# sadPororo/AD-YOLO

Hardware: AMD Instinct MI355X
Metric: train-step audio-sec/s (4ch, se-resnet34+adyolo) (higher is better)
Workload: dtype f32; 1 GPU; se-resnet34 + adyolo loss, synthetic 4ch 24kHz 60s clips, bs=64 per GPU, 12 classes, features+fwd+loss+bwd+allreduce+Adam; global_batch=64, parallelism=dp1

## Files before the change

ad-yolo_amd/_lib.py:

```python
import ctypes
import os

_HERE = os.path.dirname(os.path.abspath(__file__))
LIB_PATH = os.environ.get("ADYOLO_LIB") or os.path.join(_HERE, "libadyolo_hip.so")

P = ctypes.c_void_p
I = ctypes.c_int
L = ctypes.c_long
F = ctypes.c_float
U64 = ctypes.c_uint64

SIGNATURES = {
    "adyolo_abi_version": (I, []),
    "adyolo_last_error": (ctypes.c_char_p, []),
    "adyolo_feat_stft_mel": (I, [P] * 8 + [I, I] + [P] * 4 + [I, I, I, P]),
    "adyolo_feat_finish": (I, [P] * 4 + [I, I, I, P]),
    "adyolo_feat_gcc_phat": (I, [P] * 6 + [I, I, I, I, P]),
    "adyolo_nchw_to_nhwc8": (I, [P, P, I, I, I, I, P]),
    "adyolo_pack_w3x3": (I, [P, P, P, I, I, I, P]),
    "adyolo_conv3x3_tiles": (I, [I] * 3),
    "adyolo_conv3x3_fwd": (I, [P] * 13 + [I] * 7 + [P]),
    "adyolo_wino_pack_w": (I, [P, P, P, I, I, I, P]),
    "adyolo_wino_pack_many": (I, [P, I, I, I, P]),
    "adyolo_wino_tiles": (I, [I] * 3),
    "adyolo_wino_fwd": (I, [P] * 13 + [I] * 7 + [P]),
    "adyolo_wino4_pack_w": (I, [P, P, P, I, I, I, P]),
    "adyolo_wino4_pack_many": (I, [P, I, I, I, P]),
    "adyolo_wino4_tiles": (I, [I] * 3),
    "adyolo_wino4_fwd": (I, [P] * 13 + [I] * 7 + [P]),
    "adyolo_wino4_fwd_form": (I, [I] * 3),
    "adyolo_wino4_last_form": (I, []),
    "adyolo_set_switches": (I, [I]),
    "adyolo_wino4_wgrad_slabs": (I, [I] * 5),
    "adyolo_wino4_wgrad": (I, [P] * 7 + [I] * 6 + [P]),
    "adyolo_wino_wgrad_slabs": (I, [I] * 5),
    "adyolo_wino_wgrad": (I, [P] * 7 + [I] * 6 + [P]),
    "adyolo_conv3x3_wgrad_slabs": (I, [I] * 5),
    "adyolo_conv3x3_wgrad": (I, [P] * 6 + [I] * 6 + [P]),
    "adyolo_wgrad_plan": (I, [I] * 6 + [P]),
    "adyolo_conv_fwd_plan": (I, [I] * 9 + [P]),
    "adyolo_gemm": (I, [P] * 5 + [I] * 10 + [P]),
    "adyolo_gemm_plan": (I, [I] * 8 + [P, P, P]),
    "adyolo_gemm_batched": (I, [P] * 3 + [I] * 10 + [L] * 6 + [F, I, P]),
    "adyolo_colsum": (I, [P, P, P, I, I, I, I, P]),
    "adyolo_bn_stats": (I, [P] * 7 + [I, I, I, F, F, P]),
    "adyolo_bn_stats_tiles": (I, [P] * 11 + [I, I, I, I, F, F, P]),
    "adyolo_bn_eval_stats": (I, [P] * 4 + [I, F, P]),
    "adyolo_bn_scale_shift": (I, [P] * 6 + [I, P]),
    "adyolo_affine_nhwc": (I, [P] * 4 + [L, I, P]),
    "adyolo_bn_bwd_reduce": (I, [P] * 7 + [L, I, P]),
    "adyolo_bn_bwd_tiles": (I, [P, P, P, P, I, I, P]),
    "adyolo_bn_bwd_apply": (I, [P] * 12 + [L, I, I, F, P]),
    "adyolo_bn_persample": (I, [P, P, P, I, I, I, P]),
    "adyolo_bn_finish": (I, [P] * 10 + [I, I, I, F, F, P]),
    "adyolo_se_fc_fwd": (I, [P] * 10 + [I, I, I, I, P]),
    "adyolo_relu_mask_words": (L, [I, I, I]),
    "adyolo_se_tail_fwd": (I, [P] * 9 + [I, I, I, P]),
    "adyolo_se_tail_fwd_pool_ok": (I, [I, I, I]),
    "adyolo_se_tail_fwd_pool": (I, [P] * 9 + [I, I, I, I, P]),
    "adyolo_se_tail_bwd_reduce": (I, [P] * 9 + [I, I, I, P]),
    "adyolo_se_tail_bwd_tiles": (I, [P, P, P, I, I, I, P]),
    "adyolo_se_fc_bwd_words": (L, [I, I]),
    "adyolo_se_fc_bwd": (I, [P] * 16 + [I, I, I, I, P]),
    "adyolo_se_tail_bwd_apply": (I, [P] * 13 + [I, I, I, F, P]),
    "adyolo_se_tail_bwd_reduce_pooled": (I, [P] * 8 + [I, I, I, I, P]),
    "adyolo_se_tail_bwd_apply_pooled": (I, [P] * 13 + [I, I, I, I, F, P]),
    "adyolo_avgpool2_fwd": (I, [P, P, I, I, I, I, P]),
    "adyolo_avgpool2_bwd": (I, [P, P, I, I, I, I, P]),
    "adyolo_add": (I, [P, P, P, L, P]),
    "adyolo_mul": (I, [P, P, P, L, P]),
    "adyolo_scale_dev": (I, [P, P, P, L, P]),
    "adyolo_sap_fwd": (I, [P] * 5 + [I, I, I, P]),
    "adyolo_sap_bwd": (I, [P] * 8 + [I, I, I, P]),
    "adyolo_gru_fwd": (I, [P] * 6 + [I, I, P]),
    "adyolo_gru_bwd": (I, [P] * 6 + [I, I, P]),
    "adyolo_ln_tanh_fwd": (I, [P] * 4 + [L, I, F, P]),
    "adyolo_ln_tanh_bwd": (I, [P] * 8 + [L, I, F, P]),
    "adyolo_dropout_mask": (I, [P, L, F, U64, U64, P]),
    "adyolo_dropout_apply": (I, [P, P, L, F, U64, U64, P]),
    "adyolo_dropout_apply_dev": (I, [P, P, L, F, U64, U64, P, P]),
    "adyolo_counter_add": (I, [P, U64, P]),
    "adyolo_loss_workspace_words": (L, [I, I, I, I]),
    "adyolo_loss_fwd_bwd": (I, [P] * 6 + [I] * 7 + [P, P, F, F, F, F, P]),
    "adyolo_loss_phase": (I, [P] * 6 + [I] * 7 + [P, P, F, F, F, F, I, L, P]),
    "adyolo_loss_per_clip_workspace_words": (L, [I, I, I, I]),
    "adyolo_loss_per_clip": (I, [P] * 7 + [I] * 6 + [L, P, P, F, F, F, P]),
    "adyolo_loss_accumulate": (I, [P, P, I, P, P]),
    "adyolo_yolo_decode": (I, [P, P, L, I, I, I, I, F, F, F, P]),
    "adyolo_yolo_select_workspace_words": (L, [L, I, I]),
    "adyolo_yolo_select": (I, [P] * 4 + [L, I, I, F, F, F, F, I, P]),
    "adyolo_seld_score_workspace_words": (L, [L, I, I, I]),
# ... 120 lines not shown
```

ad-yolo_amd/csrc/conv.hip:

```cpp
#include <stdlib.h>
#include "common.hpp"

namespace adyolo {

template <int KC, int BN, int TW>
struct ConvCfg {
    static constexpr int TH = 256 / TW;
    static constexpr int HW_ = TW + 2;
    static constexpr int HH_ = TH + 2;
    static constexpr int NPIX = HW_ * HH_;
    static constexpr int AS = KC + 4;
    static constexpr int NT = BN / 32;
    static constexpr int Q = KC / 4;
    static constexpr int A_FLOATS = NPIX * AS;
    static constexpr int W_FLOATS = BN * AS;
    static constexpr int WPT = (BN * Q + 255) / 256;
};

template <int KC, int BN, int TW>
__global__ __launch_bounds__(256, 2) void conv3x3_fwd_kernel(
    const float *__restrict__ x, const float *__restrict__ wpk, const float *__restrict__ bias,
    const float *__restrict__ addend, const float *__restrict__ addend_mask, const float *__restrict__ in_scale,
    const float *__restrict__ in_shift, float *__restrict__ y, float *__restrict__ stats,
    const float *__restrict__ stat_aux, const float *__restrict__ stat_mean, const float *__restrict__ stat_invstd,
// ... 352 lines not shown
        f32x16 acc;
#pragma unroll
        for (int r = 0; r < 16; ++r) acc[r] = 0.f;
#pragma unroll
        for (int tap = 0; tap < 9; ++tap) {
            acc = mfma32(a[tap].x, bw[tap].x, acc);
            acc = mfma32(a[tap].y, bw[tap].y, acc);
            acc = mfma32(a[tap].z, bw[tap].z, acc);
            acc = mfma32(a[tap].w, bw[tap].w, acc);
        }
        if (gy < H) {
            float *ot = otile[wave];
#pragma unroll
            for (int r = 0; r < 16; ++r) {
                const int px = mfma_row(r, lane);
                float v = acc[r] + bv;
                if (relu) v = fmaxf(v, 0.f);
                ot[px * 36 + li] = v;
                if (tx0 + px < W) {
                    ssum += v;
                    float sq = v * v;
                    asm volatile("" : "+v"(sq));
                    ssq += sq;
                }
            }
            float *yrow = y + (((size_t)n * H + gy) * W + tx0) * 32;
#pragma unroll
            for (int k = 0; k < 4; ++k) {
                const int px = k * 8 + (lane >> 3), c4 = lane & 7;
                const f32x4 v4 = *reinterpret_cast<const f32x4 *>(&ot[px * 36 + c4 * 4]);
                if (tx0 + px < W) __builtin_nontemporal_store(v4, reinterpret_cast<f32x4 *>(yrow + (size_t)px * 32 + c4 * 4));
            }
        }
    }
    if (stats) {
        const float a0 = ssum + __shfl_xor(ssum, 32, 64), a1 = ssq + __shfl_xor(ssq, 32, 64);
        if (lh == 0) {
            red[(wave * 32 + li) * 2 + 0] = a0;
            red[(wave * 32 + li) * 2 + 1] = a1;
        }
        __syncthreads();
        if (tid < 64) {
            const int c = tid >> 1, which = tid & 1;
            const float v = red[(0 * 32 + c) * 2 + which] + red[(1 * 32 + c) * 2 + which] + red[(2 * 32 + c) * 2 + which] +
                            red[(3 * 32 + c) * 2 + which];
            stats[which * ((size_t)gridDim.x * 32) + (size_t)blockIdx.x * 32 + c] = v;
        }
    }
}

constexpr int SW_U = 8;
constexpr int SW_T = 64;
constexpr int SW_XS = (SW_T + 4) * 8;
__global__ __launch_bounds__(256, 2) void stem_wgrad_kernel(const float *__restrict__ x, const float *__restrict__ dy,
                                                            float *__restrict__ slabs, int H, int W, int rows_total) {
    __shared__ __attribute__((aligned(16))) float lds[4 * SW_T * 32 + 7 * SW_XS];
    static_assert(4 * SW_T * 32 + 7 * SW_XS >= 4 * 32 * 72, "the reduction buffer must fit");
    float *dyL = lds, *xL = lds + 4 * SW_T * 32;
    const int tid = threadIdx.x, lane = tid & 63, wave = tid >> 6;
    const int li = lane & 31, lh = lane >> 5;
    int ky[3], boff[3];
#pragma unroll
    for (int t = 0; t < 3; ++t) {
        const int n = t * 32 + li, tap = n < 72 ? n >> 3 : 8;
        ky[t] = tap / 3 - 1;
        boff[t] = (lh + 1 + (tap % 3 - 1)) * 8 + (n & 7);
    }
    f32x16 acc[3];
#pragma unroll
    for (int t = 0; t < 3; ++t)
#pragma unroll
        for (int r = 0; r < 16; ++r) acc[t][r] = 0.f;
    for (int i = tid; i < SW_XS; i += 256) xL[6 * SW_XS + i] = 0.f;

    const int per = (rows_total + gridDim.x - 1) / gridDim.x;
    const int r0 = blockIdx.x * per, r1 = min(rows_total, r0 + per);
    const int ncol = (W + SW_T - 1) / SW_T;
    const int nchunk = r0 < r1 ? ((r1 - r0 + 3) / 4) * ncol : 0;
    f32x4 pd[8], px_[4];
    auto request = [&](int chunk) {
        const int cr = r0 + (chunk / ncol) * 4, c0 = (chunk % ncol) * SW_T;
        const __amdgpu_buffer_rsrc_t drs = __builtin_amdgcn_make_buffer_rsrc(const_cast<float *>(dy) + (size_t)cr * W * 32, 0,
                                                                              0x7fffffff, 0x00020000);
        const __amdgpu_buffer_rsrc_t xrs = __builtin_amdgcn_make_buffer_rsrc(const_cast<float *>(x) + ((ptrdiff_t)cr - 1) * W * 8, 0,
                                                                              0x7fffffff, 0x00020000);
#pragma unroll
        for (int i = 0; i < 8; ++i) {
            const int f = tid + 256 * i;
            const int j = f >> 9, col = c0 + ((f & 511) >> 3);
            const bool ok = cr + j < r1 && col < W;
            pd[i] = __builtin_bit_cast(f32x4, __builtin_amdgcn_raw_buffer_load_b128(
                                                  drs, ok ? ((j * W + col) * 32 + (f & 7) * 4) * 4 : (int)0x80000000, 0, 0));
        }
#pragma unroll
        for (int i = 0; i < 4; ++i) {
            const int f = tid + 256 * i;
            const int j = f / 132, rem = f - j * 132;
            const int row = cr - 1 + j, col = c0 - 1 + (rem >> 1);
            const bool ok = f < 6 * 132 && row >= 0 && row < rows_total && col >= 0 && col < W;
            px_[i] = __builtin_bit_cast(f32x4, __builtin_amdgcn_raw_buffer_load_b128(
                                                   xrs, ok ? ((j * W + col) * 8 + (rem & 1) * 4) * 4 : (int)0x80000000, 0, 0));
        }
    };
    auto deposit = [&]() {
#pragma unroll
        for (int i = 0; i < 8; ++i) *reinterpret_cast<f32x4 *>(&dyL[(tid + 256 * i) * 4]) = pd[i];
#pragma unroll
        for (int i = 0; i < 4; ++i) {
            const int f = tid + 256 * i;
            const int j = f / 132;
            if (f < 6 * 132) *reinterpret_cast<f32x4 *>(&xL[j * SW_XS + (f - j * 132) * 4]) = px_[i];
        }
    };
    if (nchunk > 0) request(0);
    for (int chunk = 0; chunk < nchunk; ++chunk) {
        deposit();
        __syncthreads();
        if (chunk + 1 < nchunk) request(chunk + 1);
        const int row = r0 + (chunk / ncol) * 4 + wave;
        if (row < r1) {
            const int y = row % H;
            const float *ap = dyL + (wave * SW_T + lh) * 32 + li;
            const float *bp[3];
#pragma unroll
            for (int t = 0; t < 3; ++t) {
                const int yy = y + ky[t];
                bp[t] = xL + ((yy >= 0 && yy < H) ? wave + 1 + ky[t] : 6) * SW_XS + boff[t];
            }
            constexpr int NG = SW_T / (2 * SW_U);
            float a[2][SW_U], b[2][3][SW_U];
            auto reads = [&](int g) {
#pragma unroll
                for (int u = 0; u < SW_U; ++u) {
                    a[g & 1][u] = ap[(g * SW_U + u) * 64];
#pragma unroll
                    for (int t = 0; t < 3; ++t) b[g & 1][t][u] = bp[t][(g * SW_U + u) * 16];
                }
            };
            reads(0);
#pragma unroll
            for (int g = 0; g < NG; ++g) {
                __builtin_amdgcn_sched_barrier(0);
                if (g + 1 < NG) reads(g + 1);
                __builtin_amdgcn_sched_barrier(0);
#pragma unroll
                for (int u = 0; u < SW_U; ++u)
#pragma unroll
                    for (int t = 0; t < 3; ++t) acc[t] = mfma32(a[g & 1][u], b[g & 1][t][u], acc[t]);
            }
        }
        __syncthreads();
    }
    float *red = lds;
#pragma unroll
    for (int t = 0; t < 3; ++t)
#pragma unroll
        for (int r = 0; r < 16; ++r) {
            const int n = t * 32 + li;
            if (n < 72) red[(wave * 32 + mfma_row(r, lane)) * 72 + n] = acc[t][r];
        }
    __syncthreads();
    for (int i = tid; i < 32 * 72; i += 256)
        slabs[(size_t)blockIdx.x * (32 * 72) + i] = ((red[i] + red[32 * 72 + i]) + red[2 * 32 * 72 + i]) + red[3 * 32 * 72 + i];
}

__global__ __launch_bounds__(256) void conv3x3_wgrad_reduce_kernel(const float *__restrict__ slabs,
                                                                   float *__restrict__ dw, int nslab, int Cout,
                                                                   int CinP, int Cin_real) {
    __shared__ double red[256];
    const int total = Cout * 9 * CinP;
    const double sum = block_colsum32(slabs, nslab, (size_t)total, blockIdx.x * 32, total, red);
    const int idx = blockIdx.x * 32 + (threadIdx.x & 31);
    if ((threadIdx.x >> 5) != 0 || idx >= total) return;
    const int ci = idx % CinP;
    const int tap = (idx / CinP) % 9;
    const int co = idx / (CinP * 9);
    if (ci < Cin_real) dw[((size_t)co * Cin_real + ci) * 9 + tap] = (float)sum;
}

__global__ void pack_w3x3_kernel(const float *__restrict__ w, float *__restrict__ wf,
                                 float *__restrict__ wd, int Cout, int Cin_real, int Cin) {
    const int idx = blockIdx.x * blockDim.x + threadIdx.x;
    if (idx >= Cout * 9 * Cin) return;
    const int ci = idx % Cin;
    const int tap = (idx / Cin) % 9;
    const int co = idx / (Cin * 9);
    const float v = ci < Cin_real ? w[((size_t)co * Cin_real + ci) * 9 + tap] : 0.f;
    wf[idx] = v;
    if (wd) wd[((size_t)ci * 9 + (8 - tap)) * Cout + co] = v;
}

template <int KC, int BN, int TW>
static int launch_fwd(const float *x, const float *wpk, const float *bias, const float *addend,
                      const float *addend_mask, const float *in_scale, const float *in_shift, float *y, float *stats,
                      const float *stat_aux, const float *stat_mean, const float *stat_invstd, const float *stat_mask,
                      int N, int H, int W, int Cin, int Cout, int relu, int mask_bits, hipStream_t st, int tilesW, int tilesH) {
    dim3 grid((unsigned)(N * tilesH * tilesW), (unsigned)(Cout / BN));
    hipLaunchKernelGGL((conv3x3_fwd_kernel<KC, BN, TW>), grid, dim3(256), 0, st, x, wpk, bias, addend, addend_mask,
                       in_scale, in_shift, y, stats, stat_aux, stat_mean, stat_invstd, stat_mask, H, W, Cin, Cout, tilesW,
                       tilesH, relu, mask_bits);
    return check_launch("conv3x3_fwd");
}

static int wgrad_splits(int N, int H, int W, int Cin, int Cout, int *TWo) {
    const int TW = W >= 32 ? 32 : 16, TH = 256 / TW;
    const int ntiles = N * cdiv(H, TH) * cdiv(W, TW);
    const int blocks = (Cout / 32) * cdiv(Cin, 32);
    int nsplit = 1024 / blocks;
    if (nsplit < 1) nsplit = 1;
    if (nsplit > ntiles) nsplit = ntiles;
    if (TWo) *TWo = TW;
    return nsplit;
}

}

// ... 29 lines not shown
    v.tilesW = cdiv(W, v.TW);
    v.tilesH = cdiv(H, v.TH);
    return v;
}

extern "C" int adyolo_conv3x3_fwd(const float *x, const float *wpk, const float *bias, const float *addend,
                                  const float *addend_mask, const float *in_scale, const float *in_shift, float *y,
                                  float *stats, const float *stat_aux, const float *stat_mean,
                                  const float *stat_invstd, const float *stat_mask, int N, int H, int W, int Cin,
                                  int Cout, int relu, int mask_bits, void *stream) {
    ADYOLO_REQUIRE(x && wpk && y && N > 0 && H > 0 && W > 0, ADYOLO_EINVAL, "conv3x3_fwd: bad arguments");
    ADYOLO_REQUIRE(!(mask_bits & ~3) && (!mask_bits || ((long)H * W * (Cout / 4)) % 64 == 0), ADYOLO_ENOSUP,
                   "conv3x3_fwd: mask bits need H*W*Cout/4 %% 64 == 0");
    ADYOLO_REQUIRE((Cin == 8 || Cin % 32 == 0) && Cout % 32 == 0, ADYOLO_ENOSUP,
                   "conv3x3_fwd: Cin=%d must be 8 or a multiple of 32, Cout=%d a multiple of 32", Cin, Cout);
    ADYOLO_REQUIRE((in_scale == nullptr) == (in_shift == nullptr) && (!addend_mask || addend), ADYOLO_EINVAL,
                   "conv3x3_fwd: in_scale/in_shift come together; addend_mask needs addend");
    ADYOLO_REQUIRE(!stat_aux || (stats && stat_mean && stat_invstd), ADYOLO_EINVAL,
                   "conv3x3_fwd: stat_aux needs stats, stat_mean and stat_invstd");
    ADYOLO_REQUIRE(!stat_mask || stats, ADYOLO_EINVAL, "conv3x3_fwd: stat_mask needs stats");
    hipStream_t st = as_stream(stream);
    const ConvFwdVariant v = conv3x3_fwd_variant(H, W, Cin, Cout, !addend && !in_scale && !stat_aux && !stat_mask);
#define ADYOLO_FWD(KC_, BN_, TW_) \
    launch_fwd<KC_, BN_, TW_>(x, wpk, bias, addend, addend_mask, in_scale, in_shift, y, stats, stat_aux, stat_mean, \
                              stat_invstd, stat_mask, N, H, W, Cin, Cout, relu, mask_bits, st, v.tilesW, v.tilesH)
    if (v.stem) {
        hipLaunchKernelGGL(stem_fwd_kernel, dim3((unsigned)(N * v.tilesH * v.tilesW)), dim3(256), 0, st, x, wpk, bias, y, stats, H,
                           W, v.tilesW, v.tilesH, relu);
        return check_launch("stem_fwd");
    }
    const bool wide = v.TW == 32;
    if (v.KC == 8) return wide ? ADYOLO_FWD(8, 32, 32) : ADYOLO_FWD(8, 32, 16);
    if (v.BN == 64) return wide ? ADYOLO_FWD(32, 64, 32) : ADYOLO_FWD(32, 64, 16);
    return wide ? ADYOLO_FWD(32, 32, 32) : ADYOLO_FWD(32, 32, 16);
#undef ADYOLO_FWD
}

extern "C" int adyolo_conv3x3_wgrad_slabs(int N, int H, int W, int Cin, int Cout) {
    if (N <= 0 || H <= 0 || W <= 0 || Cin <= 0 || Cout <= 0 || Cout % 32) return ADYOLO_EINVAL;
    return wgrad_splits(N, H, W, Cin, Cout, nullptr);
}

extern "C" int adyolo_conv3x3_wgrad(const float *x, const float *dy, const float *in_scale, const float *in_shift,
                                    float *slabs, float *dw, int N, int H, int W, int Cin, int Cin_real, int Cout,
                                    void *stream) {
    ADYOLO_REQUIRE(x && dy && slabs && dw && N > 0 && H > 0 && W > 0, ADYOLO_EINVAL, "conv3x3_wgrad: bad arguments");
    ADYOLO_REQUIRE((Cin == 8 || Cin % 32 == 0) && Cout % 32 == 0 && Cin_real <= Cin, ADYOLO_ENOSUP,
                   "conv3x3_wgrad: unsupported channels Cin=%d Cout=%d", Cin, Cout);
    hipStream_t st = as_stream(stream);
    int TW;
    const int nsplit = wgrad_splits(N, H, W, Cin, Cout, &TW);
    if (Cin == 8 && Cout == 32 && !in_scale && (long)N * H < (1L << 31)) {
        const int nblk = nsplit < 512 ? nsplit : 512;
        hipLaunchKernelGGL(stem_wgrad_kernel, dim3(nblk), dim3(256), 0, st, x, dy, slabs, H, W, N * H);
        int rcs = check_launch("stem_wgrad");
        if (rcs) return rcs;
        hipLaunchKernelGGL(conv3x3_wgrad_reduce_kernel, dim3(cdiv(32 * 72, 32)), dim3(256), 0, st, slabs, dw, nblk, 32, 8,
                           Cin_real);
        return check_launch("stem_wgrad_reduce");
    }
    const int TH = 256 / TW;
    const int tilesW = cdiv(W, TW), tilesH = cdiv(H, TH);
    const int ntiles = N * tilesW * tilesH;
    const int cinBlocks = cdiv(Cin, 32);
    dim3 grid((unsigned)nsplit, (unsigned)((Cout / 32) * cinBlocks));
    if (TW == 32)
        hipLaunchKernelGGL((conv3x3_wgrad_kernel<32>), grid, dim3(256), 0, st, x, dy, in_scale, in_shift, slabs, H, W,
                           Cin, Cout, tilesW, tilesH, ntiles, nsplit, cinBlocks);
    else
        hipLaunchKernelGGL((conv3x3_wgrad_kernel<16>), grid, dim3(256), 0, st, x, dy, in_scale, in_shift, slabs, H, W,
                           Cin, Cout, tilesW, tilesH, ntiles, nsplit, cinBlocks);
    int rc = check_launch("conv3x3_wgrad");
    if (rc) return rc;
    const int CinP = cinBlocks * 32;
    const int total = Cout * 9 * CinP;
    hipLaunchKernelGGL(conv3x3_wgrad_reduce_kernel, dim3(cdiv(total, 32)), dim3(256), 0, st, slabs, dw, nsplit,
                       Cout, CinP, Cin_real);
    return check_launch("conv3x3_wgrad_reduce");
}

extern "C" int adyolo_wgrad_plan(int form, int N, int H, int W, int Cin, int Cout, int *out8) {
    ADYOLO_REQUIRE(out8 && form >= 0 && form <= 3 && N > 0 && H > 0 && W > 0 && Cin > 0 && Cout > 0, ADYOLO_EINVAL,
                   "wgrad_plan: bad arguments");
    for (int i = 0; i < 8; ++i) out8[i] = 0;
    if (form <= 1) {
        if (Cout % 32 || (Cin != 8 && Cin % 32)) return 0;
        if (form == 1 && !(Cin == 8 && Cout == 32 && (long)N * H < (1L << 31))) return 0;
        int TW;
        const int nsplit = wgrad_splits(N, H, W, Cin, Cout, &TW);
        out8[0] = nsplit;
        out8[2] = 1;
        out8[4] = 1;
        if (form == 0) {
            out8[1] = N * cdiv(H, 256 / TW) * cdiv(W, TW);
            out8[3] = 256 / TW;
            out8[5] = TW;
        } else {
            const int nblk = nsplit < 512 ? nsplit : 512;
            out8[1] = N * H;
            out8[3] = cdiv(N * H, nblk);
            out8[5] = SW_T;
            out8[6] = nblk;
        }
        out8[7] = 1;
        return 0;
    }
    if (form == 2) {
        if (adyolo_wino_wgrad_slabs(N, H, W, Cin, Cout) <= 0 ||
            (size_t)H * W * (Cin > Cout ? Cin : Cout) * 4 >= ((size_t)1 << 31))
            return 0;
        wino_wgrad_plan(N, H, W, Cin, Cout, out8);
    } else {
        if (adyolo_wino4_wgrad_slabs(N, H, W, Cin, Cout) <= 0) return 0;
        wino4_wgrad_plan(N, H, W, Cin, Cout, out8);
    }
    out8[7] = 1;
    return 0;
}

extern "C" int adyolo_conv_fwd_plan(int form, int N, int H, int W, int Cin, int Cout, int operands, int mask_bits, int affine,
                                    int *out24) {
    ADYOLO_REQUIRE(out24 && form >= 0 && form <= 3 && N > 0 && H > 0 && W > 0 && Cin > 0 && Cout > 0 && operands >= 0 && operands < 64,
                   ADYOLO_EINVAL, "conv_fwd_plan: bad arguments");
    for (int i = 0; i < 24; ++i) out24[i] = 0;
    if ((mask_bits & ~3) || (mask_bits && ((long)H * W * (Cout / 4)) % 64 != 0)) return 0;
    if (((operands & ADYOLO_W4_ADDEND_MASK) && !(operands & ADYOLO_W4_ADDEND)) ||
        ((operands & (ADYOLO_W4_STAT_AUX | ADYOLO_W4_STAT_MASK)) && !(operands & ADYOLO_W4_STATS)))
        return 0;
    if (form <= 1) {
        if (Cout % 32 || (Cin != 8 && Cin % 32)) return 0;
        const ConvFwdVariant v = conv3x3_fwd_variant(
// ... 53 lines not shown
```

ad-yolo_amd/functional.py:

```python
import os
from typing import NamedTuple

import torch

from . import ops

FUSE_BNBWD = os.environ.get("ADYOLO_FUSE_BNBWD", "1") != "0"
FUSE_POOL = os.environ.get("ADYOLO_FUSE_POOL", "1") != "0"
FUSE_POOL_BWD = os.environ.get("ADYOLO_FUSE_POOL_BWD", "1") != "0"


class BlockLink:

    def __init__(self):
        self.cc = self.mean2 = self.invstd2 = self.tiles = self.ebits = None
        self.affine = self.stem_bn = None
        self.prepooled = None


class BlockArgs(NamedTuple):
    bn1: object
    bn2: object
    bnd: object = None
    link_in: object = None
# ... 137 lines not shown
        return c[1:]

    def stats_tiles(self, tile_stats, x, update=True, affine=None):
        m = self.mod
        n, c = x.shape[0], x.shape[-1]
        hw = x.numel() // (n * c)
        g, b = affine if affine is not None else (None, None)
        if update:
            ops.params_changed()
            out = ops.bn_stats_tiles(tile_stats, n, hw, m.running_mean, m.running_var, m.momentum, m.eps, g, b)
            _bump_counter(m.num_batches_tracked)
            return out
        return ops.bn_stats_tiles(tile_stats, n, hw, None, None, m.momentum, m.eps, g, b)


class StemFn(torch.autograd.Function):

    @staticmethod
    def forward(ctx, x8, w, b, gamma, beta, bn, training, holder=None):
        wpk, _ = ops.pack_w3x3(w, x8.shape[-1], want_dgrad=False)
        if training:
            a, st = ops.conv3x3(x8, wpk, w.shape[0], bias=b, relu=True, want_stats=True)
            _, mean, invstd, scale, shift = _BNState(bn).stats_tiles(st, a, affine=(gamma, beta))
        else:
            a = ops.conv3x3(x8, wpk, w.shape[0], bias=b, relu=True)
            mean, invstd, scale, shift = _BNState(bn).eval_affine(gamma, beta)
        ctx.holder = None
        if holder is not None:
            holder.affine = (scale, shift)
            if training and FUSE_BNBWD:
                holder.stem_bn = (a.detach(), mean, invstd)
                ctx.holder = holder
            out = a
        else:
            out = ops.affine(a, scale, shift)
        ctx.training = training
        ctx.cin_real = w.shape[1]
        ctx.ptrs = (w.data_ptr(), gamma.data_ptr(), beta.data_ptr())
        ctx.wshape = tuple(w.shape)
        ctx.saved_names = ["x8", "a", "gamma", "mean", "invstd"]
        ctx.save_for_backward(x8, a, gamma, mean, invstd)
        return out

    @staticmethod
    def backward(ctx, dout):
        if not ctx.training:
            raise NotImplementedError("backward through eval-mode BatchNorm is not part of the hot path")
        x8, a, gamma, mean, invstd = ctx.saved_tensors
        pw, pg, pb = ctx.ptrs
        vg, vb, vw = SINK.view(pg), SINK.view(pb), SINK.view(pw, ctx.wshape)
        tiles = None
        if ctx.holder is not None and ctx.holder.tiles is not None:
            tiles, ctx.holder.tiles = ctx.holder.tiles, None
        da, dgamma, dbeta, db = ops.bn_bwd(_c(dout), a, gamma, mean, invstd, relu_mask=True, tile_stats=tiles,
                                           out_dgamma=vg, out_dbeta=vb, want_dx_colsum=True)
        dw = ops.conv3x3_wgrad(x8, da, ctx.cin_real, out=vw)
        if vw is not None:
            SINK.done(pw, pg, pb)
            return None, None, db, None, None, None, None, None
        return None, dw, db, dgamma, dbeta, None, None, None


class SEBlockFn(torch.autograd.Function):

    @staticmethod
    def forward(ctx, x, training, pool, args, w1, g1, b1, w2, g2, b2, fw1, fb1, fw2, fb2, wd=None, gd=None, bd=None):
        link_in, link_out, p_aff = args.link_in, args.link_out, args.in_affine
        prepooled = pool and link_in is not None and link_in.prepooled is not None
        if prepooled and tuple(x.shape[1:3]) != link_in.prepooled:
            raise ValueError("SEBlockFn: link_in.prepooled says the block below wrote a %d x %d map, but the input is %d x %d"
                             % (link_in.prepooled + tuple(x.shape[1:3])))
        if p_aff is not None and (pool or wd is not None):
            raise NotImplementedError("p_affine is only supported for identity-shortcut blocks without pooling")
        p = ops.avgpool2(x) if (pool and not prepooled) else x
        n, h, w_, cin = p.shape
        c = w1.shape[0]
        if args.packs is not None:
            wpk1, wpk1d, wpk2, wpk2d = args.packs
        else:
            wpk1, wpk1d = ops.pack_w3x3(w1, cin)
            wpk2, wpk2d = ops.pack_w3x3(w2, c)
        if training:
            a, st1 = ops.conv3x3(p, wpk1, c, relu=True, want_stats=True, in_affine=p_aff)
            _, mean1, invstd1, scale1, shift1 = _BNState(args.bn1).stats_tiles(st1, a, affine=(g1, b1))
        else:
            a = ops.conv3x3(p, wpk1, c, relu=True, in_affine=p_aff)
            mean1, invstd1, scale1, shift1 = _BNState(args.bn1).eval_affine(g1, b1)
        cc, st2 = ops.conv3x3(a, wpk2, c, in_affine=(scale1, shift1), want_stats=True)
        if training:
            ssum2, mean2, invstd2, scale2, shift2 = _BNState(args.bn2).stats_tiles(st2, cc, affine=(g2, b2))
        else:
            ssum2, _, _ = _BNState(args.bn2).stats_tiles(st2, cc, update=False)
            mean2, invstd2, scale2, shift2 = _BNState(args.bn2).eval_affine(g2, b2)
        pooled, hid, s = ops.se_fc_fwd(ssum2, scale2, shift2, fw1, fb1, fw2, fb2, h * w_)
        q = None
        meand = invstdd = None
        if wd is not None:
            q = ops.gemm(p, wd, n * h * w_, c, cin, cin, cin).view(n, h, w_, c)
            if training:
                _, meand, invstdd = _BNState(args.bnd).stats(q, True)
                scaled, shiftd = ops.bn_scale_shift(gd, bd, meand, invstdd)
            else:
                meand, invstdd, scaled, shiftd = _BNState(args.bnd).eval_affine(gd, bd)
            r, raff = q, (scaled, shiftd)
        else:
            r, raff = p, p_aff
# ... 629 lines not shown
```

ad-yolo_amd/ops.py:

```python
import ctypes
import os

import numpy as np
import torch

from . import _lib

_c = _lib.call
NULL = ctypes.c_void_p(0)


def _p(t):
    if t is None:
        return NULL
    return ctypes.c_void_p(t.data_ptr())


def _stream():
    return ctypes.c_void_p(torch.cuda.current_stream().cuda_stream)


def _chk(*ts):
    for t in ts:
        if t is None:
# ... 274 lines not shown
    stats = _new(x, 2, getattr(lib, tiles_fn)(n, h, w), cout) if want_stats else None
    sc, sh = in_affine if in_affine is not None else (None, None)
    sa, sm, si = stat_bn if stat_bn is not None else (None, None, None)
    _c(fn, _p(x), _p(wpk), _p(bias), _p(addend), _p(addend_mask),
       _p(sc), _p(sh), _p(y), _p(stats), _p(sa), _p(sm), _p(si), _p(stat_mask), n, h, w, cin, cout, int(relu), mbits,
       _stream())
    if DISPATCH_LOG is not None:
        k = (name or _W4_KERNELS[w4_form], cin, cout, epi)
        DISPATCH_LOG[k] = DISPATCH_LOG.get(k, 0) + 1
    return (y, stats) if want_stats else y


def wgrad_form(cin, cout, algo=None, shape=None):
    algo = algo or W4_THRESHOLDS["wgrad_algo"] or conv_algo()
    if algo == "winograd4" and shape is not None and cin % 32 == 0 and cout % 32 == 0:
        n, h, w = shape
        if (w % 16 == 0 or w in (4, 8)) and h % 4 == 0 and n * w // 16 * (h // 4) * cin * cout >= W4_THRESHOLDS["min_wgrad_work"] and \
                _lib.load().adyolo_wino4_wgrad_slabs(n, h, w, cin, cout) > 0:
            return "wino4_wgrad_kernel", 9.0 / 36.0
    if algo in ("winograd", "winograd4") and cin % 32 == 0 and cout % 32 == 0:
        return "wino_wgrad_kernel", 16.0 / 36.0
    return "conv3x3_wgrad_kernel", 1.0


_WGRAD_FORMS = {"wino4_wgrad_kernel": ("adyolo_wino4_wgrad", 36), "wino_wgrad_kernel": ("adyolo_wino_wgrad", 16)}


def conv3x3_wgrad(x, dy, cin_real, in_affine=None, algo=None, out=None):
    _chk(x, dy)
    n, h, w, cin = x.shape
    cout = dy.shape[3]
    sc, sh = in_affine if in_affine is not None else (None, None)
    dw = out if out is not None else _new(x, cout, cin_real, 3, 3)
    form = wgrad_form(cin, cout, algo, (n, h, w))[0]
    if DISPATCH_LOG is not None:
        k = (form, cin, cout, 1 if in_affine is not None else 0)
        DISPATCH_LOG[k] = DISPATCH_LOG.get(k, 0) + 1
    if form in _WGRAD_FORMS:
        fn, points = _WGRAD_FORMS[form]
        nslab = getattr(_lib.load(), fn + "_slabs")(n, h, w, cin, cout)
        if nslab <= 0:
            raise _lib.AdyoloHipError("%s_slabs rejected the shape" % fn)
        slabs = _new(x, nslab, points, cin, cout)
        du = _new(x, points, cin, cout)
        _c(fn, _p(x), _p(dy), _p(sc), _p(sh), _p(slabs), _p(du), _p(dw), n, h, w, cin, cin_real, cout, _stream())
        return dw
    nslab = _lib.load().adyolo_conv3x3_wgrad_slabs(n, h, w, cin, cout)
    if nslab <= 0:
        raise _lib.AdyoloHipError("conv3x3_wgrad_slabs rejected the shape")
    cinp = ((cin + 31) // 32) * 32
    slabs = _new(x, nslab, cout, 9, cinp)
    _c("adyolo_conv3x3_wgrad", _p(x), _p(dy), _p(sc), _p(sh), _p(slabs), _p(dw), n, h, w, cin, cin_real, cout, _stream())
    return dw


def gemm(a, b, m, n, k, lda, ldb, trans_a=False, trans_b=False, bias=None, out=None, ldc=None, accumulate=False,
         splits=1):
    if ldc is None:
        ldc = n
    if out is None:
        out = _new(a, m, n)
        ldc = n
    slabs = None
    if splits > 1:
        slabs = _new(a, splits, m, n)
    _c("adyolo_gemm", _p(a), _p(b), _p(bias), _p(out), _p(slabs), m, n, k, lda, ldb, ldc, int(trans_a), int(trans_b),
       splits, int(accumulate), _stream())
    return out


def wgrad_splits(m, n, k):
    tiles = ((m + 127) // 128) * ((n + 63) // 64)
    want = (512 + tiles - 1) // tiles
    return max(1, min(256, want, k // 512))


def linear(x2d, w, bias=None):
    _chk(x2d, w, bias)
    r, k = x2d.shape
    return gemm(x2d, w, r, w.shape[0], k, k, k, bias=bias)


def linear_bwd(x2d, w, dy2d, need_dx=True, out_dw=None, out_db=None, need_db=True):
    _chk(x2d, w, dy2d)
    r, k = x2d.shape
    n = w.shape[0]
    if n % 4:
        return _linear_bwd_padded(x2d, w, dy2d, need_dx, out_dw, out_db, need_db)
    dx = gemm(dy2d, w, r, k, n, n, k, trans_b=True) if need_dx else None
    dw = gemm(dy2d, x2d, n, k, r, n, k, trans_a=True, trans_b=True, splits=wgrad_splits(n, k, r), out=out_dw)
    db = colsum(dy2d, out=out_db) if need_db else None
    return dx, dw, db


def _linear_bwd_padded(x2d, w, dy2d, need_dx, out_dw, out_db, need_db):
    r, k = x2d.shape
    n = w.shape[0]
    n4 = (n + 3) // 4 * 4
    dyp = _zeros(dy2d, r, n4)
    dyp[:, :n].copy_(dy2d)
    dx = None
    if need_dx:
        wp = _zeros(w, n4, k)
        wp[:n].copy_(w)
        dx = gemm(dyp, wp, r, k, n4, n4, k, trans_b=True)
    dw = gemm(dyp, x2d, n4, k, r, n4, k, trans_a=True, trans_b=True, splits=wgrad_splits(n4, k, r))[:n]
# ... 1378 lines not shown
```

include/adyolo_hip.h:

```cpp
#ifndef ADYOLO_HIP_H
#define ADYOLO_HIP_H

#include <stddef.h>
#include <stdint.h>

#ifdef __cplusplus
extern "C" {
#endif

#define ADYOLO_ABI_VERSION 3
#define ADYOLO_EINVAL (-1)
#define ADYOLO_ENOSUP (-2)

int         adyolo_abi_version(void);
const char *adyolo_last_error(void);

int adyolo_feat_stft_mel(const float *audio, const int64_t *clip_offset, const float *twiddle,
                         const int32_t *chunk_mel, const int32_t *chunk_start, const int32_t *chunk_len,
                         const int32_t *chunk_off, const float *mel_w, int n_chunks, int n_mel_w,
                         const float *scaler_mean, const float *scaler_rstd, float *out, float *chan_max, int B,
                         int n_samples, int layout, void *stream);
int adyolo_feat_finish(float *out, const float *chan_max, const float *scaler_mean,
                       const float *scaler_rstd, int B, int T, int layout, void *stream);

int adyolo_feat_gcc_phat(const float *audio, const int64_t *clip_offset , const float *twiddle,
                         const float *scaler_mean, const float *scaler_rstd, float *out, int B, int n_samples,
                         int pix_stride, int ch0, void *stream);
int adyolo_nchw_to_nhwc8(const float *x, float *y, int B, int C, int H, int W, void *stream);

int adyolo_pack_w3x3(const float *w , float *wpk_fwd ,
                     float *wpk_dgrad , int Cout, int Cin_real, int Cin,
                     void *stream);
int adyolo_conv3x3_tiles(int N, int H, int W);
int adyolo_conv3x3_fwd(const float *x, const float *wpk, const float *bias, const float *addend,
                       const float *addend_mask, const float *in_scale, const float *in_shift, float *y,
                       float *stats, const float *stat_aux, const float *stat_mean, const float *stat_invstd,
                       const float *stat_mask, int N, int H, int W, int Cin, int Cout, int relu, int mask_bits, void *stream);
int adyolo_wino_pack_w(const float *w , float *u_fwd , float *u_dgrad ,
                       int Cout, int Cin_real, int Cin, void *stream);
int adyolo_wino_pack_many(const int64_t *table, int n, int max_cout, int max_cin, void *stream);
int adyolo_wino_tiles(int N, int H, int W);
int adyolo_wino_fwd(const float *x, const float *u, const float *bias, const float *addend,
                    const float *addend_mask, const float *in_scale, const float *in_shift, float *y, float *stats,
                    const float *stat_aux, const float *stat_mean, const float *stat_invstd, const float *stat_mask,
                    int N, int H, int W, int Cin, int Cout, int relu, int mask_bits, void *stream);
int adyolo_wino4_pack_w(const float *w , float *u_fwd , float *u_dgrad ,
                        int Cout, int Cin_real, int Cin, void *stream);
int adyolo_wino4_pack_many(const int64_t *table, int n, int max_cout, int max_cin, void *stream);
int adyolo_wino4_tiles(int N, int H, int W);
int adyolo_wino4_fwd(const float *x, const float *u, const float *bias, const float *addend, const float *addend_mask,
                     const float *in_scale, const float *in_shift, float *y, float *stats, const float *stat_aux,
                     const float *stat_mean, const float *stat_invstd, const float *stat_mask, int N, int H, int W, int Cin,
                     int Cout, int relu, int mask_bits, void *stream);
#define ADYOLO_W4_STATS 1
#define ADYOLO_W4_ADDEND 2
#define ADYOLO_W4_ADDEND_MASK 4
#define ADYOLO_W4_STAT_AUX 8
#define ADYOLO_W4_STAT_MASK 16
#define ADYOLO_W4_BIAS 32
int adyolo_wino4_fwd_form(int Cout, int operands, int mask_bits);
int adyolo_wino4_last_form(void);
int adyolo_set_switches(int bits);
int adyolo_wino4_wgrad_slabs(int N, int H, int W, int Cin, int Cout);
int adyolo_wino4_wgrad(const float *x, const float *dy, const float *in_scale , const float *in_shift ,
                       float *slabs, float *du , float *dw, int N, int H, int W, int Cin, int Cin_real,
                       int Cout, void *stream);
int adyolo_wino_wgrad_slabs(int N, int H, int W, int Cin, int Cout);
int adyolo_wino_wgrad(const float *x, const float *dy, const float *in_scale, const float *in_shift, float *slabs,
                      float *du, float *dw, int N, int H, int W, int Cin, int Cin_real, int Cout, void *stream);
int adyolo_conv3x3_wgrad_slabs(int N, int H, int W, int Cin, int Cout);
int adyolo_conv3x3_wgrad(const float *x, const float *dy, const float *in_scale, const float *in_shift,
                         float *slabs, float *dw, int N, int H, int W, int Cin, int Cin_real, int Cout,
                         void *stream);
int adyolo_wgrad_plan(int form, int N, int H, int W, int Cin, int Cout, int *out8);
int adyolo_conv_fwd_plan(int form, int N, int H, int W, int Cin, int Cout, int operands, int mask_bits, int affine, int *out24);

int adyolo_gemm(const float *A, const float *B, const float *bias, float *C, float *slabs, int M,
                int N, int K, int lda, int ldb, int ldc, int transA, int transB, int splits,
                int accumulate, void *stream);
int adyolo_gemm_plan(int M, int N, int K, int lda, int ldb, int transA, int transB, int splits, int *klen,
                     int *eff_splits, int *fastg);
int adyolo_gemm_batched(const float *A, const float *B, float *C, int M, int N, int K, int lda, int ldb, int ldc,
                        int transA, int transB, int outer, int inner, long oA, long iA, long oB, long iB, long oC,
                        long iC, float alpha, int accumulate, void *stream);
int adyolo_colsum(const float *A, float *out, float *partial, int R, int C, int lda, int accumulate,
                  void *stream);

int adyolo_bn_stats(const float *x, float *ssum, float *mean, float *invstd, float *running_mean,
                    float *running_var, float *partial, int N, int HW, int C, float momentum,
                    float eps, void *stream);
int adyolo_bn_stats_tiles(const float *tile_stats, float *ssum, float *mean, float *invstd, float *running_mean,
                          float *running_var, const float *gamma, const float *beta, float *scale, float *shift,
                          float *partial, int N, int G, int HW, int C, float momentum, float eps, void *stream);
int adyolo_bn_persample(const float *tile_stats, float *ps0, float *ps1, int N, int G, int C, void *stream);
int adyolo_bn_finish(const float *ps0, const float *ps1, float *mean, float *invstd, float *running_mean,
                     float *running_var, const float *gamma, const float *beta, float *scale, float *shift, int N,
                     int HW, int C, float momentum, float eps, void *stream);
int adyolo_bn_eval_stats(const float *running_mean, const float *running_var, float *mean,
                         float *invstd, int C, float eps, void *stream);
int adyolo_bn_scale_shift(const float *gamma, const float *beta, const float *mean,
                          const float *invstd, float *scale, float *shift, int C, void *stream);
int adyolo_affine_nhwc(const float *x, const float *scale, const float *shift, float *y, long rows,
                       int C, void *stream);
int adyolo_bn_bwd_reduce(const float *dy, const float *x, const float *mean, const float *invstd,
                         float *sdy, float *sdyx, float *partial, long rows, int C, void *stream);
int adyolo_bn_bwd_tiles(const float *tile_stats, float *sdy, float *sdyx, float *partial , int tiles, int C,
                        void *stream);
int adyolo_bn_bwd_apply(const float *dy, const float *x, const float *gamma, const float *mean,
                        const float *invstd, const float *sdy, const float *sdyx, float *dx,
                        float *dgamma, float *dbeta, float *dx_colsum ,
                        float *colsum_partial , long rows, int C, int relu_mask,
                        float count_scale ,
                        void *stream);

int adyolo_se_fc_fwd(const float *ssum, const float *scale, const float *shift, const float *w1,
                     const float *b1, const float *w2, const float *b2, float *pooled, float *hid,
                     float *s, int N, int HW, int C, int Cr, void *stream);
long adyolo_relu_mask_words(int N, int HW, int C);
int adyolo_se_tail_fwd(const float *c, const float *r, const float *scale, const float *shift,
                       const float *s, const float *r_scale , const float *r_shift , float *e,
                       uint64_t *mask , int N, int HW, int C, void *stream);
int adyolo_se_tail_fwd_pool_ok(int H, int W, int C);
int adyolo_se_tail_fwd_pool(const float *c, const float *r, const float *scale, const float *shift, const float *s,
                            const float *r_scale , const float *r_shift , float *pooled,
                            uint64_t *mask , int N, int H, int W, int C, void *stream);
int adyolo_se_tail_bwd_reduce(const float *de, const float *e, const uint64_t *mask , const float *c,
// ... 265 lines not shown
```

Before: 36530 audio-s/s.

## Fuse stem BN+ReLU backward into stem conv weight-gradient kernel

Adds a templated BN variant of the stem wgrad kernel. It computes the BN/ReLU input gradient on the fly from dy, the activations and per-channel coefficients while staging into LDS, and accumulates the bias gradient column sums in double. This removes the separate bn_bwd pass that wrote a full-resolution da tensor that the wgrad kernel then read back. In exchange the kernel loads an extra activation tensor, halves the MFMA unroll to relieve register pressure, and needs a new reduce kernel for dw and db.

```diff
diff --git a/ad-yolo_amd/_lib.py b/ad-yolo_amd/_lib.py
--- a/ad-yolo_amd/_lib.py
+++ b/ad-yolo_amd/_lib.py
@@ -37,6 +37,8 @@
     "adyolo_wino_wgrad": (I, [P] * 7 + [I] * 6 + [P]),
     "adyolo_conv3x3_wgrad_slabs": (I, [I] * 5),
     "adyolo_conv3x3_wgrad": (I, [P] * 6 + [I] * 6 + [P]),
+    "adyolo_stem_bn_wgrad_ok": (I, [I] * 5),
+    "adyolo_stem_bn_wgrad": (I, [P] * 11 + [I] * 4 + [F, P]),
     "adyolo_wgrad_plan": (I, [I] * 6 + [P]),
     "adyolo_conv_fwd_plan": (I, [I] * 9 + [P]),
     "adyolo_gemm": (I, [P] * 5 + [I] * 10 + [P]),
diff --git a/ad-yolo_amd/csrc/conv.hip b/ad-yolo_amd/csrc/conv.hip
--- a/ad-yolo_amd/csrc/conv.hip
+++ b/ad-yolo_amd/csrc/conv.hip
@@ -428,8 +428,24 @@
 constexpr int SW_U = 8;
 constexpr int SW_T = 64;
 constexpr int SW_XS = (SW_T + 4) * 8;
+
+struct StemBnArgs {
+    const float *a, *gamma, *mean, *invstd, *sdy, *sdyx;
+    float invR;
+};
+constexpr int SW_SLAB = 32 * 72;
+
+__device__ __forceinline__ float stem_bn_da(float d, float av, float gi, float ai, float m, float is, float b, float invR) {
+#pragma clang fp contract(off)
+    const float t = ((av - m) * is) * b;
+    const float o = gi * __builtin_fmaf(-invR, t, d - ai);
+    return av > 0.f ? o : 0.f;
+}
+
+template <bool BN>
 __global__ __launch_bounds__(256, 2) void stem_wgrad_kernel(const float *__restrict__ x, const float *__restrict__ dy,
-                                                            float *__restrict__ slabs, int H, int W, int rows_total) {
+                                                            float *__restrict__ slabs, int H, int W, int rows_total,
+                                                            const StemBnArgs bn) {
     __shared__ __attribute__((aligned(16))) float lds[4 * SW_T * 32 + 7 * SW_XS];
     static_assert(4 * SW_T * 32 + 7 * SW_XS >= 4 * 32 * 72, "the reduction buffer must fit");
     float *dyL = lds, *xL = lds + 4 * SW_T * 32;
@@ -453,20 +469,38 @@
     const int r0 = blockIdx.x * per, r1 = min(rows_total, r0 + per);
     const int ncol = (W + SW_T - 1) / SW_T;
     const int nchunk = r0 < r1 ? ((r1 - r0 + 3) / 4) * ncol : 0;
-    f32x4 pd[8], px_[4];
+    f32x4 pd[8], px_[4], pa[BN ? 8 : 1];
+    __shared__ __attribute__((aligned(16))) float coef[BN ? 5 * 32 : 4];
+    double sacc[4] = {0.0, 0.0, 0.0, 0.0};
+    if constexpr (BN) {
+#pragma clang fp contract(off)
+        if (tid < 32) {
+            const float is = bn.invstd[tid];
+            coef[0 * 32 + tid] = bn.gamma[tid] * is;
+            coef[1 * 32 + tid] = bn.sdy[tid] * bn.invR;
+            coef[2 * 32 + tid] = bn.mean[tid];
+            coef[3 * 32 + tid] = is;
+            coef[4 * 32 + tid] = bn.sdyx[tid];
+        }
+        __syncthreads();
+    }
     auto request = [&](int chunk) {
         const int cr = r0 + (chunk / ncol) * 4, c0 = (chunk % ncol) * SW_T;
         const __amdgpu_buffer_rsrc_t drs = __builtin_amdgcn_make_buffer_rsrc(const_cast<float *>(dy) + (size_t)cr * W * 32, 0,
                                                                               0x7fffffff, 0x00020000);
         const __amdgpu_buffer_rsrc_t xrs = __builtin_amdgcn_make_buffer_rsrc(const_cast<float *>(x) + ((ptrdiff_t)cr - 1) * W * 8, 0,
                                                                               0x7fffffff, 0x00020000);
+        const __amdgpu_buffer_rsrc_t ars = __builtin_amdgcn_make_buffer_rsrc(
+            const_cast<float *>(BN ? bn.a : dy) + (size_t)cr * W * 32, 0, 0x7fffffff, 0x00020000);
 #pragma unroll
         for (int i = 0; i < 8; ++i) {
             const int f = tid + 256 * i;
             const int j = f >> 9, col = c0 + ((f & 511) >> 3);
             const bool ok = cr + j < r1 && col < W;
-            pd[i] = __builtin_bit_cast(f32x4, __builtin_amdgcn_raw_buffer_load_b128(
-                                                  drs, ok ? ((j * W + col) * 32 + (f & 7) * 4) * 4 : (int)0x80000000, 0, 0));
+            const int off = ok ? ((j * W + col) * 32 + (f & 7) * 4) * 4 : (int)0x80000000;
+            pd[i] = __builtin_bit_cast(f32x4, __builtin_amdgcn_raw_buffer_load_b128(drs, off, 0, 0));
+            if constexpr (BN)
+                pa[i] = __builtin_bit_cast(f32x4, __builtin_amdgcn_raw_buffer_load_b128(ars, off, 0, 0));
         }
 #pragma unroll
         for (int i = 0; i < 4; ++i) {
@@ -479,13 +513,32 @@
         }
     };
     auto deposit = [&]() {
-#pragma unroll
-        for (int i = 0; i < 8; ++i) *reinterpret_cast<f32x4 *>(&dyL[(tid + 256 * i) * 4]) = pd[i];
+        f32x4 gi, ai, cm, cis, cb;
+        float cs[4] = {0.f, 0.f, 0.f, 0.f};
+        if constexpr (BN) {
+            const f32x4 *cq = reinterpret_cast<const f32x4 *>(coef) + (tid & 7);
+            gi = cq[0], ai = cq[8], cm = cq[16], cis = cq[24], cb = cq[32];
+        }
+#pragma unroll
+        for (int i = 0; i < 8; ++i) {
+            if constexpr (BN) {
+#pragma unroll
+                for (int k = 0; k < 4; ++k) {
+                    pd[i][k] = stem_bn_da(pd[i][k], pa[i][k], gi[k], ai[k], cm[k], cis[k], cb[k], bn.invR);
+                    cs[k] += pd[i][k];
+                }
+            }
+            *reinterpret_cast<f32x4 *>(&dyL[(tid + 256 * i) * 4]) = pd[i];
+        }
 #pragma unroll
         for (int i = 0; i < 4; ++i) {
             const int f = tid + 256 * i;
             const int j = f / 132;
             if (f < 6 * 132) *reinterpret_cast<f32x4 *>(&xL[j * SW_XS + (f - j * 132) * 4]) = px_[i];
+        }
+        if constexpr (BN) {
+#pragma unroll
+            for (int k = 0; k < 4; ++k) sacc[k] += (double)cs[k];
         }
     };
     if (nchunk > 0) request(0);
@@ -503,14 +556,14 @@
                 const int yy = y + ky[t];
                 bp[t] = xL + ((yy >= 0 && yy < H) ? wave + 1 + ky[t] : 6) * SW_XS + boff[t];
             }
-            constexpr int NG = SW_T / (2 * SW_U);
-            float a[2][SW_U], b[2][3][SW_U];
+            constexpr int U = BN ? SW_U / 2 : SW_U, NG = SW_T / (2 * U);
+            float a[2][U], b[2][3][U];
             auto reads = [&](int g) {
 #pragma unroll
-                for (int u = 0; u < SW_U; ++u) {
-                    a[g & 1][u] = ap[(g * SW_U + u) * 64];
-#pragma unroll
-                    for (int t = 0; t < 3; ++t) b[g & 1][t][u] = bp[t][(g * SW_U + u) * 16];
+                for (int u = 0; u < U; ++u) {
+                    a[g & 1][u] = ap[(g * U + u) * 64];
+#pragma unroll
+                    for (int t = 0; t < 3; ++t) b[g & 1][t][u] = bp[t][(g * U + u) * 16];
                 }
             };
             reads(0);
@@ -520,7 +573,7 @@
                 if (g + 1 < NG) reads(g + 1);
                 __builtin_amdgcn_sched_barrier(0);
 #pragma unroll
-                for (int u = 0; u < SW_U; ++u)
+                for (int u = 0; u < U; ++u)
 #pragma unroll
                     for (int t = 0; t < 3; ++t) acc[t] = mfma32(a[g & 1][u], b[g & 1][t][u], acc[t]);
             }
@@ -536,8 +589,35 @@
             if (n < 72) red[(wave * 32 + mfma_row(r, lane)) * 72 + n] = acc[t][r];
         }
     __syncthreads();
-    for (int i = tid; i < 32 * 72; i += 256)
-        slabs[(size_t)blockIdx.x * (32 * 72) + i] = ((red[i] + red[32 * 72 + i]) + red[2 * 32 * 72 + i]) + red[3 * 32 * 72 + i];
+    float *slab = slabs + (size_t)blockIdx.x * (SW_SLAB + (BN ? 32 : 0));
+    for (int i = tid; i < 32 * 72; i += 256) slab[i] = ((red[i] + red[32 * 72 + i]) + red[2 * 32 * 72 + i]) + red[3 * 32 * 72 + i];
+    if constexpr (BN) {
+        __syncthreads();
+        double *dred = reinterpret_cast<double *>(lds);
+#pragma unroll
+        for (int k = 0; k < 4; ++k) dred[tid * 4 + k] = sacc[k];
+        __syncthreads();
+        if (tid < 32) {
+            double t = dred[tid];
+            for (int j = 1; j < 32; ++j) t += dred[j * 32 + tid];
+            slab[SW_SLAB + tid] = (float)t;
+        }
+    }
+}
+
+__global__ __launch_bounds__(256) void stem_bn_wgrad_reduce_kernel(const float *__restrict__ slabs, float *__restrict__ dw,
+                                                                   float *__restrict__ db, int nslab, int Cin_real) {
+    __shared__ double red[256];
+    const int total = SW_SLAB + 32;
+    const double sum = block_colsum32(slabs, nslab, (size_t)total, blockIdx.x * 32, total, red);
+    const int idx = blockIdx.x * 32 + (threadIdx.x & 31);
+    if ((threadIdx.x >> 5) != 0 || idx >= total) return;
+    if (idx >= SW_SLAB) {
+        db[idx - SW_SLAB] = (float)sum;
+        return;
+    }
+    const int ci = idx % 8, tap = (idx / 8) % 9, co = idx / 72;
+    if (ci < Cin_real) dw[((size_t)co * Cin_real + ci) * 9 + tap] = (float)sum;
 }
 
 __global__ __launch_bounds__(256) void conv3x3_wgrad_reduce_kernel(const float *__restrict__ slabs,
@@ -673,7 +753,7 @@
     const int nsplit = wgrad_splits(N, H, W, Cin, Cout, &TW);
     if (Cin == 8 && Cout == 32 && !in_scale && (long)N * H < (1L << 31)) {
         const int nblk = nsplit < 512 ? nsplit : 512;
-        hipLaunchKernelGGL(stem_wgrad_kernel, dim3(nblk), dim3(256), 0, st, x, dy, slabs, H, W, N * H);
+        hipLaunchKernelGGL(stem_wgrad_kernel<false>, dim3(nblk), dim3(256), 0, st, x, dy, slabs, H, W, N * H, StemBnArgs{});
         int rcs = check_launch("stem_wgrad");
         if (rcs) return rcs;
         hipLaunchKernelGGL(conv3x3_wgrad_reduce_kernel, dim3(cdiv(32 * 72, 32)), dim3(256), 0, st, slabs, dw, nblk, 32, 8,
@@ -698,6 +778,28 @@
     hipLaunchKernelGGL(conv3x3_wgrad_reduce_kernel, dim3(cdiv(total, 32)), dim3(256), 0, st, slabs, dw, nsplit,
                        Cout, CinP, Cin_real);
     return check_launch("conv3x3_wgrad_reduce");
+}
+
+extern "C" int adyolo_stem_bn_wgrad_ok(int N, int H, int W, int Cin, int Cout) {
+    return N > 0 && H > 0 && W > 0 && W <= (1 << 20) && Cin == 8 && Cout == 32 && (long)N * H < (1L << 31);
+}
+
+extern "C" int adyolo_stem_bn_wgrad(const float *x, const float *dy, const float *a, const float *gamma, const float *mean,
+                                    const float *invstd, const float *sdy, const float *sdyx, float *slabs, float *dw, float *db,
+                                    int N, int H, int W, int Cin_real, float count_scale, void *stream) {
+    ADYOLO_REQUIRE(x && dy && a && gamma && mean && invstd && sdy && sdyx && slabs && dw && db && Cin_real > 0 && Cin_real <= 8 &&
+                       count_scale >= 1.f,
+                   ADYOLO_EINVAL, "stem_bn_wgrad: bad arguments");
+    ADYOLO_REQUIRE(adyolo_stem_bn_wgrad_ok(N, H, W, 8, 32), ADYOLO_ENOSUP, "stem_bn_wgrad: unsupported shape");
+    hipStream_t st = as_stream(stream);
+    const int nsplit = wgrad_splits(N, H, W, 8, 32, nullptr);
+    const int nblk = nsplit < 512 ? nsplit : 512;
+    const StemBnArgs bn = {a, gamma, mean, invstd, sdy, sdyx, (float)(1.0 / ((double)N * H * W * (double)count_scale))};
+    hipLaunchKernelGGL(stem_wgrad_kernel<true>, dim3(nblk), dim3(256), 0, st, x, dy, slabs, H, W, N * H, bn);
+    int rc = check_launch("stem_bn_wgrad");
+    if (rc) return rc;
+    hipLaunchKernelGGL(stem_bn_wgrad_reduce_kernel, dim3(cdiv(SW_SLAB + 32, 32)), dim3(256), 0, st, slabs, dw, db, nblk, Cin_real);
+    return check_launch("stem_bn_wgrad_reduce");
 }
 
 extern "C" int adyolo_wgrad_plan(int form, int N, int H, int W, int Cin, int Cout, int *out8) {
diff --git a/ad-yolo_amd/functional.py b/ad-yolo_amd/functional.py
--- a/ad-yolo_amd/functional.py
+++ b/ad-yolo_amd/functional.py
@@ -213,6 +213,14 @@
         tiles = None
         if ctx.holder is not None and ctx.holder.tiles is not None:
             tiles, ctx.holder.tiles = ctx.holder.tiles, None
+        n, h, w, cin = x8.shape
+        if tiles is not None and ops.stem_bn_wgrad_ok(n, h, w, cin, a.shape[-1]):
+            dw, db, dgamma, dbeta = ops.stem_bn_wgrad(x8, _c(dout), a, gamma, mean, invstd, ctx.cin_real, tile_stats=tiles,
+                                                      out=vw, out_dgamma=vg, out_dbeta=vb)
+            if vw is not None:
+                SINK.done(pw, pg, pb)
+                return None, None, db, None, None, None, None, None
+            return None, dw, db, dgamma, dbeta, None, None, None
         da, dgamma, dbeta, db = ops.bn_bwd(_c(dout), a, gamma, mean, invstd, relu_mask=True, tile_stats=tiles,
                                            out_dgamma=vg, out_dbeta=vb, want_dx_colsum=True)
         dw = ops.conv3x3_wgrad(x8, da, ctx.cin_real, out=vw)
diff --git a/ad-yolo_amd/ops.py b/ad-yolo_amd/ops.py
--- a/ad-yolo_amd/ops.py
+++ b/ad-yolo_amd/ops.py
@@ -350,6 +350,42 @@
     slabs = _new(x, nslab, cout, 9, cinp)
     _c("adyolo_conv3x3_wgrad", _p(x), _p(dy), _p(sc), _p(sh), _p(slabs), _p(dw), n, h, w, cin, cin_real, cout, _stream())
     return dw
+
+
+def stem_bn_wgrad_ok(n, h, w, cin, cout):
+    return bool(_lib.load().adyolo_stem_bn_wgrad_ok(int(n), int(h), int(w), int(cin), int(cout)))
+
+
+def stem_bn_wgrad(x, dy, a, gamma, mean, invstd, cin_real, tile_stats=None, out=None, out_dgamma=None, out_dbeta=None):
+    _chk(x, dy, a, gamma, mean, invstd)
+    n, h, w, cin = x.shape
+    c = a.shape[-1]
+    if tuple(a.shape) != (n, h, w, c) or dy.shape != a.shape:
+        raise _lib.AdyoloHipError("stem_bn_wgrad: dy and a must be [N][H][W][C] over x's pixels")
+    sdy = out_dbeta if out_dbeta is not None else _new(a, c)
+    sdyx = out_dgamma if out_dgamma is not None else _new(a, c)
+    if tile_stats is not None:
+        _c("adyolo_bn_bwd_tiles", _p(tile_stats), _p(sdy), _p(sdyx), _p(_new(tile_stats, 2, 256, c)), tile_stats.shape[1], c,
+           _stream())
+    else:
+        _c("adyolo_bn_bwd_reduce", _p(dy), _p(a), _p(mean), _p(invstd), _p(sdy), _p(sdyx), _p(_new(a, 2 * 1024 * c)), n * h * w, c,
+           _stream())
+    a_sdy, a_sdyx, cs = sdy, sdyx, 1.0
+    if EXACT.on:
+        glob = EXACT.all_reduce(torch.stack([sdy, sdyx]))
+        a_sdy, a_sdyx, cs = glob[0], glob[1], float(EXACT.world)
+    dw = out if out is not None else _new(x, c, cin_real, 3, 3)
+    db = _new(a, c)
+    if DISPATCH_LOG is not None:
+        k = ("conv3x3_wgrad_kernel", cin, c, 0)
+        DISPATCH_LOG[k] = DISPATCH_LOG.get(k, 0) + 1
+    nslab = _lib.load().adyolo_conv3x3_wgrad_slabs(n, h, w, cin, c)
+    if nslab <= 0 or not stem_bn_wgrad_ok(n, h, w, cin, c):
+        raise _lib.AdyoloHipError("stem_bn_wgrad: unsupported shape")
+    slabs = _new(x, nslab, 32 * 72 + 32)
+    _c("adyolo_stem_bn_wgrad", _p(x), _p(dy), _p(a), _p(gamma), _p(mean), _p(invstd), _p(a_sdy), _p(a_sdyx), _p(slabs), _p(dw),
+       _p(db), n, h, w, cin_real, cs, _stream())
+    return dw, db, sdyx, sdy
 
 
 def gemm(a, b, m, n, k, lda, ldb, trans_a=False, trans_b=False, bias=None, out=None, ldc=None, accumulate=False,
diff --git a/include/adyolo_hip.h b/include/adyolo_hip.h
--- a/include/adyolo_hip.h
+++ b/include/adyolo_hip.h
@@ -72,6 +72,10 @@
 int adyolo_conv3x3_wgrad(const float *x, const float *dy, const float *in_scale, const float *in_shift,
                          float *slabs, float *dw, int N, int H, int W, int Cin, int Cin_real, int Cout,
                          void *stream);
+int adyolo_stem_bn_wgrad_ok(int N, int H, int W, int Cin, int Cout);
+int adyolo_stem_bn_wgrad(const float *x, const float *dy, const float *a, const float *gamma, const float *mean,
+                         const float *invstd, const float *sdy, const float *sdyx, float *slabs, float *dw, float *db, int N,
+                         int H, int W, int Cin_real, float count_scale, void *stream);
 int adyolo_wgrad_plan(int form, int N, int H, int W, int Cin, int Cout, int *out8);
 int adyolo_conv_fwd_plan(int form, int N, int H, int W, int Cin, int Cout, int operands, int mask_bits, int affine, int *out24);
 
```

Measured after the change: 36710 audio-s/s, median of 6. No clear change (+0.5%).
